# iris1997jiatong/I-DCCRN-VAE

Measured on AMD Instinct MI355X. Metric: 4s@16kHz utterances/sec fwd+SI-SNR, DCCRN-CL, 1/2/4/8 MI355X vs host CPU, higher is better.
Workload: dtype f32; 1 GPU; supervised DCCRN-CL forward(train=False) + final_ete_loss (weights 0/0/1); batch_per_gpu=64, utterance=4 s @ 16 kHz (64000 samples, 641 frames), parallelism=replicas x1, streams=1, input=resident in HBM

## Files before the change

### i-dccrn-vae_amd/csrc/cgemm_tw.hip

```cpp
#include <atomic>
#include <cstdint>
#include <cstdlib>
#include <type_traits>
#include "cgemm.hpp"
#include "conv_epilogue.hpp"
#include "cgemm_tw_map.hpp"
#include "../../include/idccrn_hip.h"

namespace {

struct TwArgs {
    const float* x0;
    const float* x1;
    int C0, C1;
    int Fin, Fout;
    int J, Jp, Tp;
    const float* wfrag;
    int UP;
    const float* epi;
    int has_fold;
    const float* slope;
    float* out;
    int Cout, cotiles;
    int tshift, t_valid;
    double* stats;
    int stats_rep;
    const float* add;
    int add_div, add_Jp;
    TwGrid grid;
    int stagger;
};

constexpr int TW_PACK_CI = 8;
constexpr int TW_XCD_SPLIT = 1;
constexpr int TW_PAIR_STAGGER = 1;

template <int PH> __device__ __forceinline__ int tw_ra(int r) {
    if (PH == 0) return r == 0 ? 0 : (r == 2 ? 2 : 1);
    return r == 0 ? 1 : 2;
}
template <int PH> __device__ __forceinline__ int tw_rb(int r) {
    if (PH == 0) return r == 2 ? 1 : (r == 3 ? 3 : 2);
    return r == 0 ? 2 : 3;
}
template <int PH> __device__ __forceinline__ float tw_cb(int r) {
    if (PH == 0) return r == 1 ? 1.f : -1.f;
    return r == 1 ? 0.f : -1.f;
}
template <int PH> constexpr int tw_nr() { return PH == 0 ? 4 : 3; }
template <int PH> constexpr int tw_nt() { return tw_nr<PH>() * 9; }
template <int PH> constexpr int tw_ntp() { return PH == 0 ? 36 : 32; }
template <int PH> constexpr int tw_ntw() { return (tw_nt<PH>() + 3) / 4; }
__host__ __device__ inline int tw_tile(int ph, int w, int k) {
    if (ph == 0) return w * 9 + k;
    if (w < 3) return k < 6 ? w * 9 + k : w * 9 + 8;
    return k < 6 ? (k >> 1) * 9 + 6 + (k & 1) : -1;
}
template <int PH> constexpr int tw_wslots() { return PH == 0 ? 9 : 8; }

template <int PH, int CIK, bool LEFT, bool STATS = false, int NCT = 1>
__global__ __launch_bounds__(256 * NCT, NCT == 1 ? 2 : 1) void cconv_tw_kernel(const TwArgs a) {
    constexpr int NR = tw_nr<PH>(), NT = tw_nt<PH>(), NTP = tw_ntp<PH>(), NTW = tw_ntw<PH>();
    constexpr int NRAW = PH == 0 ? 4 : 3, ROW0 = PH == 0 ? 0 : 1;
    constexpr int KS = CIK / 2;
    constexpr int RT = NRAW * 9 * 32;
    constexpr int NE = CIK * RT;
    constexpr int NBUF = 2;
    constexpr int RDW = 2;
    constexpr bool STAGE_BEHIND_W = PH == 0 && NCT == 2;
    constexpr int NITEM = CIK * NRAW * 16;
    constexpr int NTHR = 256 * NCT;
    constexpr int NLD = (NITEM + NTHR - 1) / NTHR;
    static_assert(NCT == 1 || NCT == 2, "one or two co tiles per workgroup");
    static_assert(KS % RDW == 0 && NLD <= 2, "weight ring slots are compile-time; at most two staging items per thread");
    static_assert(NLD + NCT - 1 < KS, "the staging k-steps (from 1 on, waves 4 .. 7 one later) end before the barrier's k-step");
    static_assert(NCT * NT * 4 * 64 <= NBUF * NE, "the epilogue exchange (one area per co tile) fits the patch buffers");

    extern __shared__ __attribute__((aligned(16))) float smem[];

    const int tid = threadIdx.x;
    const int lane = tid & 63;
    const int wave = __builtin_amdgcn_readfirstlane(tid >> 6);
    const int w4 = NCT == 1 ? wave : wave & 3, cth = NCT == 1 ? 0 : wave >> 2;
    const int half = lane >> 5, l31 = lane & 31;

    TwTile tile;
    if (!tw_block_tile(a.grid, blockIdx.x, tile)) return;
    const bool edge = PH == 0 && tile.edge;
    const int jt = tile.jt, ft = tile.ft;
    int ct = tile.ct;
    ct = NCT * ct + cth;
    const int j0 = jt * 64;
    const int m0 = 2 * ft;
    const int rbase = m0 - 1 + ROW0;

    const int Cin = a.C0 + a.C1;
    const int nchunk = (Cin + CIK - 1) / CIK;

    f32x16 acc[NTW];
#pragma unroll
    for (int k = 0; k < NTW; ++k)
#pragma unroll
        for (int r = 0; r < 16; ++r) acc[k][r] = 0.f;
    constexpr int NPAIR = (NTW - 1) / 2;
    constexpr bool UNI = PH == 0;
    int offA[UNI ? 1 : NPAIR + 1], offB[UNI ? 1 : NPAIR + 1];
    float cbj[UNI ? 1 : NPAIR + 1];
    if (UNI) {
        cbj[0] = edge ? 0.f : tw_cb<PH>(w4);
        offA[0] = (edge ? w4 : tw_ra<PH>(w4) - ROW0) * 288;
        offB[0] = (edge ? w4 : tw_rb<PH>(w4) - ROW0) * 288;
    } else {
#pragma unroll
        for (int j = 0; j <= NPAIR; ++j) {
            int t = tw_tile(PH, w4, j < NPAIR ? 2 * j : NTW - 1);
            t = t < 0 ? 0 : t;
            const int r = t / 9, plane = t - r * 9;
            cbj[j] = tw_cb<PH>(r);
            const int po = plane == 8 ? 256 : (plane >> 1) * 64;
            offA[j] = (tw_ra<PH>(r) - ROW0) * 288 + po;
            offB[j] = cbj[j] != 0.f ? (tw_rb<PH>(r) - ROW0) * 288 + po : offA[j];
        }
    }

    f32x4 v_r[NLD], v_i[NLD];
    float e_r[NLD], e_i[NLD];
    unsigned off_v[NLD], off_e[NLD], ldsoff[NLD];
    unsigned okmask[NLD];
    int item_cl[NLD];
    bool interior[NLD];
#pragma unroll
    for (int i = 0; i < NLD; ++i) {
        const int e = tid + i * NTHR;
        const int c8 = e & 15;
        const int rl = (e >> 4) % NRAW, cl = e / (16 * NRAW);
        item_cl[i] = cl;
        const int f = edge ? a.Fin - 2 + (rl & 1) : rbase + rl;
        const int jc = j0 + (edge ? 64 * (rl >> 1) : 0) + 4 * c8;
        const int je = LEFT ? jc - 1 : jc + 4;
        const bool exists = e < NITEM;
        const bool okr = exists && f >= 0 && f < a.Fin;
        unsigned m = 0;
#pragma unroll
        for (int q = 0; q < 5; ++q) {
            const int c = jc + q + (LEFT ? -1 : 0);
            if (c >= 0 && c < a.J) m |= 1u << q;
        }
        if (okr) m |= 1u << 5;
        if (exists) m |= 1u << 7;
        const int jcv = jc + 3 < a.Jp ? jc : 0;
        const int jev = (je >= 0 && je < a.Jp) ? je : 0;
        off_v[i] = okr ? (unsigned)((cl * a.Fin + f) * a.Jp + jcv) : 0u;
        off_e[i] = okr ? (unsigned)((cl * a.Fin + f) * a.Jp + jev) : 0u;
        if (jc + 3 >= a.Jp) m &= ~0x1fu;
        if (!(je >= 0 && je < a.Jp)) m &= LEFT ? ~1u : ~(1u << 4);
        okmask[i] = m;
        interior[i] = __builtin_amdgcn_ballot_w64((m & 0xbfu) == 0xbfu) == ~0ull;
        ldsoff[i] = (unsigned)((cl * NRAW + rl) * 288 + 4 * c8);
    }
    auto stage_load = [&](int chunk, int i) {
        const int ci0 = chunk * CIK;
        const bool from0 = ci0 < a.C0;
        const float* br = from0 ? a.x0 + (size_t)ci0 * a.Fin * a.Jp : a.x1 + (size_t)(ci0 - a.C0) * a.Fin * a.Jp;
        const float* bi = from0 ? br + (size_t)a.C0 * a.Fin * a.Jp : br + (size_t)a.C1 * a.Fin * a.Jp;
        const int cvalid = (from0 ? a.C0 : Cin) - ci0;
        const bool dead = item_cl[i] >= cvalid;
        const unsigned ov = dead ? 0u : off_v[i], oe = dead ? 0u : off_e[i];
        v_r[i] = *(const f32x4*)(br + ov);
        v_i[i] = *(const f32x4*)(bi + ov);
        e_r[i] = br[oe];
        e_i[i] = bi[oe];
    };
    float fr[5], fi[5];
    auto stage_window = [&](int chunk, int i) {
        const int ci0s = chunk * CIK;
        const int cvalid = (ci0s < a.C0 ? a.C0 : Cin) - ci0s;
        constexpr bool left = LEFT;
        if (interior[i] && cvalid >= CIK) {
#pragma unroll
            for (int q = 0; q < 5; ++q) {
                fr[q] = left ? (q == 0 ? e_r[i] : v_r[i][q == 0 ? 0 : q - 1]) : (q == 4 ? e_r[i] : v_r[i][q == 4 ? 3 : q]);
                fi[q] = left ? (q == 0 ? e_i[i] : v_i[i][q == 0 ? 0 : q - 1]) : (q == 4 ? e_i[i] : v_i[i][q == 4 ? 3 : q]);
            }
            return;
        }
        unsigned m = okmask[i];
        if (item_cl[i] >= cvalid || !((m >> 5) & 1u)) m &= ~0x1fu;
#pragma unroll
        for (int q = 0; q < 5; ++q) {
            const float xr = left ? (q == 0 ? e_r[i] : v_r[i][q == 0 ? 0 : q - 1]) : (q == 4 ? e_r[i] : v_r[i][q == 4 ? 3 : q]);
            const float xi = left ? (q == 0 ? e_i[i] : v_i[i][q == 0 ? 0 : q - 1]) : (q == 4 ? e_i[i] : v_i[i][q == 4 ? 3 : q]);
            const bool cok = (m >> q) & 1u;
            fr[q] = cok ? xr : 0.f;
            fi[q] = cok ? xi : 0.f;
        }
    };
    auto plane_val = [&](int gt, int pr) -> float {
        const int g = gt / 3, tau = gt - g * 3;
        const int q0 = 2 * pr;
        const float xa_ = g == 0 ? fr[q0] + fi[q0] : (g == 1 ? fr[q0] : fi[q0]);
        const float xb_ = g == 0 ? fr[q0 + 1] + fi[q0 + 1] : (g == 1 ? fr[q0 + 1] : fi[q0 + 1]);
        const float xd_ = g == 0 ? fr[q0 + 2] + fi[q0 + 2] : (g == 1 ? fr[q0 + 2] : fi[q0 + 2]);
        return tau == 0 ? xa_ - xb_ : (tau == 1 ? xb_ : xb_ - xd_);
    };
// ... 1 lines not shown
    auto stage_plane2 = [&](float* dst, int i, int j) {
        if (!item_exists(i)) return;
        if (j < 4) {
            f32x4 o = {plane_val(2 * j, 0), plane_val(2 * j + 1, 0), plane_val(2 * j, 1), plane_val(2 * j + 1, 1)};
            *(f32x4*)(dst + ldsoff[i] + j * 64) = o;
        } else {
            *(float2*)(dst + ldsoff[i] - 2 * (int)(tid & 15) + 256) = make_float2(plane_val(8, 0), plane_val(8, 1));
        }
    };
    auto stage_store = [&](float* dst, int chunk, int i) {
        stage_window(chunk, i);
#pragma unroll
        for (int j = 0; j < 5; ++j) stage_plane2(dst, i, j);
    };

    constexpr int WS = tw_wslots<PH>();
    constexpr int NWR = PH == 0 ? NTW : 8;
    const size_t wregion = PH == 1 ? (size_t)a.cotiles * a.UP * tw_ntp<0>() : (edge ? (size_t)a.cotiles * a.UP * (tw_ntp<0>() + tw_ntp<1>()) : 0);
    const float* wbase = a.wfrag + (wregion + (size_t)ct * a.UP * NTP) * 64 + (size_t)w4 * WS * 64;
    const int total_ks = nchunk * KS;
    float a_w[RDW][NWR];
    auto load_w = [&](int g, float (&dst)[NWR]) {
        g = g < total_ks ? g : total_ks - 1;
        const float* ws = wbase + (size_t)g * NTP * 64;
        const f32x4 w0 = *(const f32x4*)(ws + lane * 4), w1 = *(const f32x4*)(ws + 256 + lane * 4);
#pragma unroll
        for (int k = 0; k < 4; ++k) {
            dst[k] = w0[k];
            dst[4 + k] = w1[k];
        }
        if (NTW == 9) dst[NTW - 1] = ws[512 + lane];
    };
    float xa[NTW], xb[NTW];
    auto load_raw2 = [&](const float* base, int j) {
        if (j < NPAIR) {
            const int oa = UNI ? offA[0] + j * 64 : offA[UNI ? 0 : j], ob = UNI ? offB[0] + j * 64 : offB[UNI ? 0 : j];
            const float2 pa_ = *(const float2*)(base + oa + 2 * l31), pb_ = *(const float2*)(base + ob + 2 * l31);
            xa[2 * j] = pa_.x; xa[2 * j + 1] = pa_.y;
            xb[2 * j] = pb_.x; xb[2 * j + 1] = pb_.y;
        } else {
            xa[NTW - 1] = base[(UNI ? offA[0] + 256 : offA[UNI ? 0 : NPAIR]) + l31];
            xb[NTW - 1] = base[(UNI ? offB[0] + 256 : offB[UNI ? 0 : NPAIR]) + l31];
        }
    };
    auto load_raw_all = [&](const float* base) {
#pragma unroll
        for (int j = 0; j <= NPAIR; ++j) load_raw2(base, j);
    };

#pragma unroll
    for (int i = 0; i < NLD; ++i) stage_load(0, i);
#pragma unroll
    for (int u = 0; u < RDW; ++u) load_w(u, a_w[u]);
#pragma unroll
    for (int i = 0; i < NLD; ++i) stage_store(smem, 0, i);
#pragma unroll
    for (int i = 0; i < NLD; ++i) stage_load(nchunk > 1 ? 1 : 0, i);
    __syncthreads();

    load_raw_all(smem + (size_t)half * RT);
    auto run = [&](auto late_) {
        constexpr bool LATE = decltype(late_)::value;
        for (int chunk = 0; chunk < nchunk; ++chunk) {
            const float* P = smem + (chunk & 1) * NE;
            float* Pn = smem + ((chunk + 1) & 1) * NE;
            const int nxt = chunk + 1 < nchunk ? chunk + 1 : chunk, nxt2 = chunk + 2 < nchunk ? chunk + 2 : nchunk - 1;
#pragma unroll
            for (int ul = 0; ul < KS; ++ul) {
                const float* bnext = ul + 1 < KS ? P + (size_t)(2 * (ul + 1) + half) * RT : Pn + (size_t)half * RT;
                const int si = ul - 1 - (LATE ? 1 : 0);
                const bool staging = si >= 0 && si < NLD;
#pragma unroll
                for (int k = 0; k < NTW; ++k) {
                    const float b = xa[k] + cbj[UNI ? 0 : (k >> 1 < NPAIR ? k >> 1 : NPAIR)] * xb[k];
                    if (PH == 1 && k == 4)
                        asm volatile("" ::"v"(a_w[ul % RDW][4]), "v"(a_w[ul % RDW][5]), "v"(a_w[ul % RDW][6]), "v"(a_w[ul % RDW][7]));
                    acc[k] = __builtin_amdgcn_mfma_f32_32x32x2f32(a_w[ul % RDW][k], b, acc[k], 0, 0, 0);
                    if (ul == KS - 1 && k == 0) {
                        __builtin_amdgcn_sched_barrier(0);
                        __syncthreads();
                    }
                    if ((k & 1) && (k >> 1) < NPAIR) load_raw2(bnext, k >> 1);
                    if (k == NTW - 1) load_raw2(bnext, NPAIR);
                    if (staging) {
                        if (k == 0) stage_window(nxt, si);
                        if ((k & 1) && k < 6) stage_plane2(Pn, si, k >> 1);
                        if (k == (NTW == 9 ? 7 : 6)) stage_plane2(Pn, si, 3);
                        if (k == NTW - 1) stage_plane2(Pn, si, 4);
                        if (k == NTW - 1 && !STAGE_BEHIND_W) stage_load(nxt2, si);
                    }
                    __builtin_amdgcn_sched_barrier(0);
                }
                load_w(chunk * KS + ul + RDW, a_w[ul % RDW]);
                if (STAGE_BEHIND_W && staging) {
                    __builtin_amdgcn_sched_barrier(0);
                    stage_load(nxt2, si);
                }
            }
        }
    };
    if (NCT == 2 && PH == 1 && a.stagger && cth)
        run(std::integral_constant<bool, NCT == 2 && PH == 1>{});
    else
        run(std::false_type{});
    __syncthreads();

    const float slope = a.slope ? *a.slope : 1.0f;
    const bool has_act = a.slope != nullptr;
    float* E = smem + cth * (NT * 4 * 64);
    const int jAc[2] = {j0 + 2 * l31, j0 + 2 * l31 + (edge ? 64 : 0)};
    bool keep[2][2], inb[2][2];
    int ja[2][2];
#pragma unroll
    for (int c = 0; c < 2; ++c)
#pragma unroll
        for (int q = 0; q < 2; ++q) {
// ... 181 lines not shown
    const int cotiles = (Cout + 31) / 32;
    const int cpad = (cin_used + TW_PACK_CI - 1) / TW_PACK_CI * TW_PACK_CI;
    const long long n = idv_cconv_tw_wfrag_floats(Cout, cin_used);
    const unsigned blocks = (unsigned)((n + 255) / 256 > 4096 ? 4096 : (n + 255) / 256);
    hipLaunchKernelGGL(pack_cconv_tw_kernel, dim3(blocks), dim3(256), 0, (hipStream_t)stream, wino_frag, cotiles, cpad * 3, cpad / 2,
                       cin_used, tw_frag);
    return idv_launch_status();
}

extern "C" int idv_ctconv2d_tw_fwd(const float* x0, int C0, const float* x1, int C1, const float* wfrag, const float* epi, int has_fold,
                                   const float* prelu_slope, float* out, double* stats, double* stats_work, int stats_rep, int tshift,
                                   int Cout, int Fin, int B, int Tp, int Jp, int t_valid_out, const float* addend, int addend_div,
                                   int addend_Jp, void* stream) {
    if (!x0 || !wfrag || !epi || !out || C0 <= 0 || Cout <= 0 || Fin <= 0 || B <= 0 || Tp <= 1) return IDV_EINVAL;
    const EpiStatsTarget sums{stats, stats_work, stats_rep};
    if (!sums.ok()) return IDV_EINVAL;
    if (addend && (addend_div < 1 || B % addend_div || addend_Jp < (B / addend_div) * Tp)) return IDV_EINVAL;
    if (C1 > 0 && !x1) return IDV_EINVAL;
    if (tshift != 0 && tshift != -1) return IDV_EINVAL;
    if (!idv_cconv_tw_supported(C0, C1, Cout, Fin)) return IDV_EINVAL;
    if ((Jp & 3) || (reinterpret_cast<uintptr_t>(x0) & 15) || (C1 > 0 && (reinterpret_cast<uintptr_t>(x1) & 15)) ||
        (reinterpret_cast<uintptr_t>(out) & 7))
        return IDV_EINVAL;
    TwArgs a{};
    a.x0 = x0; a.x1 = x1; a.C0 = C0; a.C1 = C1;
    a.Fin = Fin; a.Fout = 2 * Fin - 1;
    a.J = B * Tp; a.Jp = Jp; a.Tp = Tp;
    a.wfrag = wfrag; a.UP = (C0 + C1 + TW_PACK_CI - 1) / TW_PACK_CI * TW_PACK_CI / 2;
    a.epi = epi; a.has_fold = has_fold; a.slope = prelu_slope; a.out = out;
    a.Cout = Cout; a.cotiles = (Cout + 31) / 32;
    a.tshift = tshift; a.t_valid = t_valid_out;
    a.add = addend; a.add_div = addend ? addend_div : 1; a.add_Jp = addend_Jp;
    if (Jp < a.J) return IDV_EINVAL;
    if ((long long)8 * Fin * (long long)Jp >= 0xffffffffLL) return IDV_EINVAL;
    hipStream_t st = (hipStream_t)stream;
    sums.set(a);
    int rc = 0;
    rc = launch_tw_ph<0, 8>(a, st);
    if (!rc) rc = launch_tw_ph<1, 8>(a, st);
    return sums.finish(rc, Cout, st);
}
```

### i-dccrn-vae_amd/csrc/cgemm_tw2.hip

```cpp
#include <cstdint>
#include <cstdlib>
#include <type_traits>
#include "cgemm.hpp"
#include "conv_epilogue.hpp"
#include "cgemm_tw_map.hpp"
#include "../../include/idccrn_hip.h"

namespace {

typedef f32x4 f32x4_a4 __attribute__((aligned(4)));

struct Tw2Args {
    const float* x0;
    int Cin;
    int Fin, Fout;
    int J, Jp, Tp;
    const float* wfrag;
    int UP;
    const float* epi;
    int has_fold;
    const float* slope;
    float* out;
    int Cout, cotiles;
    int tshift, t_valid;
    double* stats;
    int stats_rep;
    TwGrid grid;
    int stagger;
};

constexpr int TW2_PACK_CI = 8;
constexpr int TW2_XCD_SPLIT = 1;
constexpr int TW2_PAIR_STAGGER = 1;

__host__ __device__ constexpr int tw2_ra(int q) { return q == 0 ? 0 : (q == 1 ? 2 : (q == 2 ? 4 : (q == 3 ? 2 : (q == 4 ? 1 : 3)))); }
__host__ __device__ constexpr int tw2_rb(int q) { return q == 0 ? 4 : (q == 1 ? 4 : (q == 2 ? 2 : (q == 3 ? 6 : (q == 4 ? 3 : (q == 5 ? 3 : 5))))); }
__host__ __device__ constexpr float tw2_cb(int q) { return q == 1 ? 1.f : (q == 5 ? 0.f : -1.f); }
__host__ __device__ constexpr int tw2_qx(int a) { return a == 0 ? 0 : (a == 1 ? 1 : 3); }
__host__ __device__ constexpr int tw2_qy(int a) { return a == 0 ? 4 : (a == 1 ? 5 : 6); }
__host__ __device__ constexpr int tw2_main_acc(int w) { return w == 2 ? 3 : w; }
__host__ __device__ inline void tw2_slot(int w, int k, int& q, int& plane) {
// ... 51 lines not shown

    const int tid = threadIdx.x;
    const int lane = tid & 63;
    const int wave = __builtin_amdgcn_readfirstlane(tid >> 6);
    const int w4 = NCT == 1 ? wave : wave & 3, cth = NCT == 1 ? 0 : wave >> 2;
    const int half = lane >> 5, l31 = lane & 31;

    TwTile tile;
    if (!tw_block_tile(a.grid, blockIdx.x, tile)) return;
    const bool edge = tile.edge;
    const int jt = tile.jt, ft = tile.ft;
    const int ct = NCT * tile.ct + cth;
    const int j0 = jt * 64;
    const int m0 = 2 * ft;
    const int rbase = 2 * m0 - 2;

    const int Cin = a.Cin;
    const int nchunk = (Cin + CIK - 1) / CIK;

    f32x16 acc[NACC];
#pragma unroll
    for (int k = 0; k < NACC; ++k)
#pragma unroll
        for (int r = 0; r < 16; ++r) acc[k][r] = 0.f;

    f32x4 v_r[NLD], v_i[NLD];
    float e_r[NLD], e_i[NLD];
    unsigned off_v[NLD], ldsoff[NLD];
    unsigned okmask[NLD];
    bool interior[NLD];
    auto item_cl = [&](int i) -> int { return (tid + i * NTHR) / (16 * NRAW); };
#pragma unroll
    for (int i = 0; i < NLD; ++i) {
        const int e = tid + i * NTHR;
        const int c8 = e & 15;
        const int cl = e / (16 * NRAW), rl = (NCT == 2 && e >= NITEM) ? 0 : (e >> 4) % NRAW;
        const int f = edge ? (rl < 6 ? a.Fin - 3 + rl % 3 : -1) : rbase + rl;
        const int jc = j0 + (edge && rl >= 3 ? 64 : 0) + 4 * c8;
        const int je = LEFT ? jc - 1 : jc + 4;
        const bool exists = e < NITEM;
        const bool okr = exists && f >= 0 && f < a.Fin;
        unsigned m = 0;
#pragma unroll
        for (int q = 0; q < 5; ++q) {
            const int c = jc + q + (LEFT ? -1 : 0);
            if (c >= 0 && c < a.J) m |= 1u << q;
        }
        if (okr) m |= 1u << 5;
        const int jcv = jc + 3 < a.Jp ? jc : 0;
        off_v[i] = okr ? (unsigned)((cl * a.Fin + f) * a.Jp + jcv) : 4u;
        if (jc + 3 >= a.Jp) m &= ~0x1fu;
        if (!(je >= 0 && je < a.Jp)) m &= LEFT ? ~1u : ~(1u << 4);
        okmask[i] = m;
        interior[i] = __builtin_amdgcn_ballot_w64((m & 0x3fu) == 0x3fu) == ~0ull;
        ldsoff[i] = (unsigned)((cl * NRAW + rl) * 288 + 4 * c8);
    }
    auto item_exists = [&](int i) -> bool { return i == 0 || wave * 64 + 256 < NITEM; };
    auto stage_load = [&](int chunk, int i) {
        if (!item_exists(i)) return;
        const int ci0 = chunk * CIK;
        const float* br = a.x0 + (size_t)ci0 * a.Fin * a.Jp;
        const float* bi = br + (size_t)Cin * a.Fin * a.Jp;
        const bool dead = item_cl(i) >= Cin - ci0;
        const unsigned ov = dead ? 4u : off_v[i];
        const float* pr = br + ov - (LEFT ? 1 : 0);
        const float* pi = bi + ov - (LEFT ? 1 : 0);
        using Win = std::conditional_t<LEFT, f32x4_a4, f32x4>;
        v_r[i] = *(const Win*)pr;
        v_i[i] = *(const Win*)pi;
        e_r[i] = pr[4];
        e_i[i] = pi[4];
    };
    float fr[5], fi[5];
    auto stage_window = [&](int chunk, int i) {
        if (!item_exists(i)) return;
        const int cvalid = Cin - chunk * CIK;
        if (interior[i] && cvalid >= CIK) {
#pragma unroll
            for (int q = 0; q < 5; ++q) {
                fr[q] = q == 4 ? e_r[i] : v_r[i][q == 4 ? 3 : q];
                fi[q] = q == 4 ? e_i[i] : v_i[i][q == 4 ? 3 : q];
            }
            return;
        }
        unsigned m = okmask[i];
        if (item_cl(i) >= cvalid || !((m >> 5) & 1u)) m &= ~0x1fu;
#pragma unroll
        for (int q = 0; q < 5; ++q) {
            const float xr = q == 4 ? e_r[i] : v_r[i][q == 4 ? 3 : q];
            const float xi = q == 4 ? e_i[i] : v_i[i][q == 4 ? 3 : q];
            const bool cok = (m >> q) & 1u;
            fr[q] = cok ? xr : 0.f;
            fi[q] = cok ? xi : 0.f;
        }
    };
    auto plane_val = [&](int gt, int pr) -> float {
        const int g = gt / 3, tau = gt - g * 3;
        const int q0 = 2 * pr;
        const float xa_ = g == 0 ? fr[q0] + fi[q0] : (g == 1 ? fr[q0] : fi[q0]);
// ... 2 lines not shown
        return tau == 0 ? xa_ - xb_ : (tau == 1 ? xb_ : xb_ - xd_);
    };
    auto stage_plane2 = [&](float* dst, int i, int j) {
        if (!item_exists(i)) return;
        if (j < 4) {
            f32x4 o = {plane_val(2 * j, 0), plane_val(2 * j + 1, 0), plane_val(2 * j, 1), plane_val(2 * j + 1, 1)};
            *(f32x4*)(dst + ldsoff[i] + j * 64) = o;
        } else {
            *(float2*)(dst + ldsoff[i] - 2 * (int)(tid & 15) + 256) = make_float2(plane_val(8, 0), plane_val(8, 1));
        }
    };
    auto stage_store = [&](float* dst, int chunk, int i) {
        stage_window(chunk, i);
#pragma unroll
        for (int j = 0; j < 5; ++j) stage_plane2(dst, i, j);
    };

    const float* wbase = a.wfrag + (((size_t)(edge ? a.cotiles : 0) + ct) * a.UP * 4 + w4) * 1024 + lane * 4;
    const int total_ks = nchunk * KS;
    float a_w[NSLOT];
    auto load_wg = [&](int g, int grp) {
        g = g < total_ks ? g : total_ks - 1;
        const f32x4 w4 = *(const f32x4*)(wbase + (size_t)g * 4096 + grp * 256);
#pragma unroll
        for (int k = 0; k < 4; ++k) a_w[grp * 4 + k] = w4[k];
    };

    const int am = tw2_main_acc(w4 < 3 ? w4 : 0);
    const int qxm = tw2_qx(am), qym = tw2_qy(am);
    const int rxa = tw2_ra(qxm) * 288, rxb = tw2_rb(qxm) * 288, rya = tw2_ra(qym) * 288, ryb = tw2_rb(qym) * 288;
    const float cbx = tw2_cb(qxm), cby = tw2_cb(qym);
    const int r2a = tw2_ra(2) * 288 + w4 * 64, r2b = tw2_rb(2) * 288 + w4 * 64;
    float xa[2][4], xb[2][4];
    auto load_grp_a = [&](const float* base, int g, float (&oa)[4], float (&ob)[4]) {
        if (g < 3) {
            const float2 xa_ = *(const float2*)(base + rxa + g * 64 + 2 * l31), xb_ = *(const float2*)(base + rxb + g * 64 + 2 * l31);
            const float2 ya_ = *(const float2*)(base + rya + g * 64 + 2 * l31), yb_ = *(const float2*)(base + ryb + g * 64 + 2 * l31);
            oa[0] = xa_.x; oa[2] = xa_.y; ob[0] = xb_.x; ob[2] = xb_.y;
            oa[1] = ya_.x; oa[3] = ya_.y; ob[1] = yb_.x; ob[3] = yb_.y;
        } else {
            oa[0] = base[rxa + 3 * 64 + 2 * l31]; ob[0] = base[rxb + 3 * 64 + 2 * l31];
            oa[1] = base[rya + 3 * 64 + 2 * l31]; ob[1] = base[ryb + 3 * 64 + 2 * l31];
            const float2 pa_ = *(const float2*)(base + r2a + 2 * l31), pb_ = *(const float2*)(base + r2b + 2 * l31);
            oa[2] = pa_.x; oa[3] = pa_.y; ob[2] = pb_.x; ob[3] = pb_.y;
        }
    };
    auto load_grp_b = [&](const float* base, int g, float (&oa)[4], float (&ob)[4]) {
#pragma unroll
        for (int s4 = 0; s4 < 4; ++s4) {
            int q, plane;
            tw2_slot(3, 4 * g + s4, q, plane);
            if (q < 0) continue;
            oa[s4] = base[tw2_ra(q) * 288 + tw2_poff(plane, l31)];
            ob[s4] = base[tw2_rb(q) * 288 + tw2_poff(plane, l31)];
        }
    };
    const int eoff = (w4 >> 1) * 3 * 288;
    auto load_grp_e = [&](auto odd_, const float* base, int g, float (&oa)[4]) {
#pragma unroll
        for (int s4 = 0; s4 < 4; ++s4) {
            int t, plane;
            if (!tw2_eslot(decltype(odd_)::value, 4 * g + s4, t, plane)) continue;
            oa[s4] = base[eoff + t * 288 + tw2_poff(plane, l31)];
        }
    };

    auto prologue = [&]() {
#pragma unroll
        for (int i = 0; i < NLD; ++i) stage_load(0, i);
#pragma unroll
        for (int grp = 0; grp < 4; ++grp) load_wg(0, grp);
#pragma unroll
        for (int i = 0; i < NLD; ++i) stage_store(smem, 0, i);
#pragma unroll
        for (int i = 0; i < NLD; ++i) stage_load(nchunk > 1 ? 1 : 0, i);
        __syncthreads();
    };

    auto run = [&](auto role, auto late_) {
        constexpr int ROLE = decltype(role)::value;
        constexpr bool ROLE_B = ROLE == 1, EDGE = ROLE >= 2;
        using EdgeOdd = std::integral_constant<bool, ROLE == 3>;
        prologue();
        if constexpr (EDGE) load_grp_e(EdgeOdd{}, smem + (size_t)half * RT, 0, xa[0]);
        else if (ROLE_B) load_grp_b(smem + (size_t)half * RT, 0, xa[0], xb[0]);
        else load_grp_a(smem + (size_t)half * RT, 0, xa[0], xb[0]);
        for (int chunk = 0; chunk < nchunk; ++chunk) {
            const float* P = smem + (chunk & 1) * NEB;
            float* Pn = smem + ((chunk + 1) & 1) * NEB;
            const int nxt = chunk + 1 < nchunk ? chunk + 1 : chunk, nxt2 = chunk + 2 < nchunk ? chunk + 2 : nchunk - 1;
#pragma unroll
            for (int ul = 0; ul < KS; ++ul) {
                const float* bnext = ul + 1 < KS ? P + (size_t)(2 * (ul + 1) + half) * RT : Pn + (size_t)half * RT;
                const bool staging = ul == 0;
#pragma unroll
                for (int k = 0; k < (ROLE_B ? NSLOT - 1 : NSLOT); ++k) {
                    const int g = k >> 2, s4 = k & 3;
                    float cb;
                    int ai;
                    bool product = true;
                    if (EDGE) {
                        int t, plane;
                        product = tw2_eslot(EdgeOdd::value, k, t, plane);
                        cb = 0.f;
                        ai = plane - (EdgeOdd::value ? 5 : 0);
                    } else if (ROLE_B) {
                        int q, plane;
                        tw2_slot(3, k, q, plane);
                        cb = tw2_cb(q);
                        ai = k < 12 ? k >> 1 : 6 + (k - 12);
                    } else {
                        cb = k < 14 ? ((k & 1) ? cby : cbx) : -1.f;
                        ai = k < 14 ? k >> 1 : 7 + (k - 14);
                    }
                    if ((ROLE_B || EDGE) && s4 == 0) asm volatile("" ::"v"(a_w[k]), "v"(a_w[k + 1]), "v"(a_w[k + 2]), "v"(a_w[k + 3]));
                    if (s4 == 0) {
                        const float* src = g < 3 ? P + (size_t)(2 * ul + half) * RT : bnext;
                        if (!(ul == KS - 1 && g == 3)) {
                            if constexpr (EDGE) load_grp_e(EdgeOdd{}, src, (g + 1) & 3, xa[(g + 1) & 1]);
                            else if (ROLE_B) load_grp_b(src, (g + 1) & 3, xa[(g + 1) & 1], xb[(g + 1) & 1]);
                            else load_grp_a(src, (g + 1) & 3, xa[(g + 1) & 1], xb[(g + 1) & 1]);
                        }
                    }
                    if constexpr (EDGE) {
                        if (product) acc[ai] = __builtin_amdgcn_mfma_f32_32x32x2f32(a_w[k], xa[g & 1][s4], acc[ai], 0, 0, 0);
                    } else {
                        const float b = xa[g & 1][s4] + cb * xb[g & 1][s4];
                        acc[ai] = __builtin_amdgcn_mfma_f32_32x32x2f32(a_w[k], b, acc[ai], 0, 0, 0);
                    }
                    if (ul == KS - 1 && k == 0) {
                        __builtin_amdgcn_sched_barrier(0);
                        __syncthreads();
                    }
                    if (ul == KS - 1 && k == 12) {
                        if constexpr (EDGE) load_grp_e(EdgeOdd{}, bnext, 0, xa[0]);
                        else if (ROLE_B) load_grp_b(bnext, 0, xa[0], xb[0]);
                        else load_grp_a(bnext, 0, xa[0], xb[0]);
                    }
                    if ((k & 3) == 3 || (ROLE_B && k == NSLOT - 2)) load_wg(chunk * KS + ul + 1, k >> 2);
                    if constexpr (NCT == 2) if (staging) {
                        constexpr bool late = decltype(late_)::value;
                        if (k <= 5 && !late) {
                            if (k == 0) stage_window(nxt, 0);
                            if (k >= 1) stage_plane2(Pn, 0, k - 1);
                            if (k == 5) stage_load(nxt2, 0);
                        }
                        if (k >= 8 && k <= 13 && late) {
                            if (k == 8) stage_window(nxt, 0);
                            if (k >= 9) stage_plane2(Pn, 0, k - 9);
                            if (k == 13) stage_load(nxt2, 0);
                        }
                    }
                    if constexpr (NCT == 1) if (staging) {
                        if (k == 0) stage_window(nxt, 0);
                        if (k >= 1 && k <= 5) stage_plane2(Pn, 0, k - 1);
                        if (k == 5) stage_load(nxt2, 0);
                        if (!ROLE_B) {
                            if (k == 8) stage_window(nxt, 1);
                            if (k >= 9 && k <= 13) stage_plane2(Pn, 1, k - 9);
                            if (k == 13) stage_load(nxt2, 1);
                        }
                    }
                    __builtin_amdgcn_sched_barrier(0);
                }
            }
        }
    };
    using Late = std::integral_constant<bool, NCT == 2>;
    const bool late = NCT == 2 && a.stagger && cth;
    if (edge) {
// ... 163 lines not shown
    const long long cotiles = (Cout + 31) / 32, cpad = (cin_used + TW2_PACK_CI - 1) / TW2_PACK_CI * TW2_PACK_CI;
    return cotiles * (cpad / 2) * 2 * 4096;
}

extern "C" int idv_pack_cconv_tw2(const float* wino_frag, int Cout, int cin_used, float* tw_frag, void* stream) {
    if (!wino_frag || !tw_frag || Cout <= 0 || cin_used <= 0) return IDV_EINVAL;
    const int cotiles = (Cout + 31) / 32;
    const int cpad = (cin_used + TW2_PACK_CI - 1) / TW2_PACK_CI * TW2_PACK_CI;
    const long long n = idv_cconv_tw2_wfrag_floats(Cout, cin_used);
    const unsigned blocks = (unsigned)((n + 255) / 256 > 4096 ? 4096 : (n + 255) / 256);
    hipLaunchKernelGGL(pack_cconv_tw2_kernel, dim3(blocks), dim3(256), 0, (hipStream_t)stream, wino_frag, cotiles, cpad * 3, cpad / 2,
                       tw_frag);
    return idv_launch_status();
}

extern "C" int idv_cconv2d_tw_fwd(const float* x0, int Cin, const float* wfrag, const float* epi, int has_fold, const float* prelu_slope,
                                  float* out, double* stats, double* stats_work, int stats_rep, int tshift, int Cout, int Fin, int B, int Tp,
                                  int Jp, int t_valid_out, void* stream) {
    if (!x0 || !wfrag || !epi || !out || Cin <= 0 || Cout <= 0 || Fin <= 0 || B <= 0 || Tp <= 1) return IDV_EINVAL;
    const EpiStatsTarget sums{stats, stats_work, stats_rep};
    if (!sums.ok()) return IDV_EINVAL;
    if (tshift != 0 && tshift != -1) return IDV_EINVAL;
    if (!idv_cconv_tw2_supported(Cin, Cout, Fin)) return IDV_EINVAL;
    if ((Jp & 3) || (reinterpret_cast<uintptr_t>(x0) & 15) || (reinterpret_cast<uintptr_t>(out) & 7)) return IDV_EINVAL;
    Tw2Args a{};
    a.x0 = x0; a.Cin = Cin;
    a.Fin = Fin; a.Fout = (Fin - 1) / 2 + 1;
    a.J = B * Tp; a.Jp = Jp; a.Tp = Tp;
    a.wfrag = wfrag; a.UP = (Cin + TW2_PACK_CI - 1) / TW2_PACK_CI * TW2_PACK_CI / 2;
    a.epi = epi; a.has_fold = has_fold; a.slope = prelu_slope; a.out = out;
    a.Cout = Cout; a.cotiles = (Cout + 31) / 32;
    a.tshift = tshift; a.t_valid = t_valid_out;
    if (Jp < a.J) return IDV_EINVAL;
    if ((long long)4 * Fin * (long long)Jp >= 0xffffffffLL) return IDV_EINVAL;
    hipStream_t st = (hipStream_t)stream;
    sums.set(a);
    int rc;
    const bool pair = a.cotiles % 2 == 0 && (idv_tw_pair(-1) & IDV_TW_PAIR_CONV);
    switch ((stats ? 4 : 0) | (pair ? 2 : 0) | (tshift ? 1 : 0)) {
        case 0: rc = launch_tw2<false, false, 1>(a, st); break;
        case 1: rc = launch_tw2<true, false, 1>(a, st); break;
        case 2: rc = launch_tw2<false, false, 2>(a, st); break;
        case 3: rc = launch_tw2<true, false, 2>(a, st); break;
        case 4: rc = launch_tw2<false, true, 1>(a, st); break;
        case 5: rc = launch_tw2<true, true, 1>(a, st); break;
        case 6: rc = launch_tw2<false, true, 2>(a, st); break;
        default: rc = launch_tw2<true, true, 2>(a, st); break;
    }
    return sums.finish(rc, Cout, st);
}
```

Before: 1059 utterances/sec.

## Use precomputed LDS base pointers, byte offsets, and one-ahead B-operand transform in tw conv kernels

The complex conv kernels now keep per-lane LDS base pointers in address space 3 and flip them between the two buffers, so operand reads can use immediate offsets instead of recomputing addresses each k-step. Global staging offsets are precomputed in bytes through a shared helper, which drops a shift per load. The B operand (xa + cb*xb) is computed one MFMA ahead so the VALU work overlaps the matrix pipe. The cost is more live registers and tighter range checks on host-side offsets.

```diff
diff --git a/i-dccrn-vae_amd/csrc/cgemm_tw.hip b/i-dccrn-vae_amd/csrc/cgemm_tw.hip
--- a/i-dccrn-vae_amd/csrc/cgemm_tw.hip
+++ b/i-dccrn-vae_amd/csrc/cgemm_tw.hip
@@ -5,9 +5,14 @@
 #include "cgemm.hpp"
 #include "conv_epilogue.hpp"
 #include "cgemm_tw_map.hpp"
+#include "cgemm_tw_stage.hpp"
 #include "../../include/idccrn_hip.h"
 
 namespace {
+
+typedef __attribute__((address_space(3))) float LdsF;
+typedef float TwF2 __attribute__((ext_vector_type(2)));
+typedef __attribute__((address_space(3))) TwF2 LdsF2;
 
 struct TwArgs {
     const float* x0;
@@ -68,6 +73,7 @@
     constexpr int NBUF = 2;
     constexpr int RDW = 2;
     constexpr bool STAGE_BEHIND_W = PH == 0 && NCT == 2;
+    constexpr bool KBASE = !(PH == 1 && NCT == 1);
     constexpr int NITEM = CIK * NRAW * 16;
     constexpr int NTHR = 256 * NCT;
     constexpr int NLD = (NITEM + NTHR - 1) / NTHR;
@@ -131,32 +137,13 @@
     bool interior[NLD];
 #pragma unroll
     for (int i = 0; i < NLD; ++i) {
-        const int e = tid + i * NTHR;
-        const int c8 = e & 15;
-        const int rl = (e >> 4) % NRAW, cl = e / (16 * NRAW);
-        item_cl[i] = cl;
-        const int f = edge ? a.Fin - 2 + (rl & 1) : rbase + rl;
-        const int jc = j0 + (edge ? 64 * (rl >> 1) : 0) + 4 * c8;
-        const int je = LEFT ? jc - 1 : jc + 4;
-        const bool exists = e < NITEM;
-        const bool okr = exists && f >= 0 && f < a.Fin;
-        unsigned m = 0;
-#pragma unroll
-        for (int q = 0; q < 5; ++q) {
-            const int c = jc + q + (LEFT ? -1 : 0);
-            if (c >= 0 && c < a.J) m |= 1u << q;
-        }
-        if (okr) m |= 1u << 5;
-        if (exists) m |= 1u << 7;
-        const int jcv = jc + 3 < a.Jp ? jc : 0;
-        const int jev = (je >= 0 && je < a.Jp) ? je : 0;
-        off_v[i] = okr ? (unsigned)((cl * a.Fin + f) * a.Jp + jcv) : 0u;
-        off_e[i] = okr ? (unsigned)((cl * a.Fin + f) * a.Jp + jev) : 0u;
-        if (jc + 3 >= a.Jp) m &= ~0x1fu;
-        if (!(je >= 0 && je < a.Jp)) m &= LEFT ? ~1u : ~(1u << 4);
-        okmask[i] = m;
-        interior[i] = __builtin_amdgcn_ballot_w64((m & 0xbfu) == 0xbfu) == ~0ull;
-        ldsoff[i] = (unsigned)((cl * NRAW + rl) * 288 + 4 * c8);
+        const TwStageItem it = tw_stage_item(tid + i * NTHR, NRAW, NITEM, LEFT, edge, a.Fin, a.J, a.Jp, j0, rbase, KBASE ? 4u : 1u);
+        item_cl[i] = it.cl;
+        off_v[i] = it.off_v;
+        off_e[i] = it.off_e;
+        okmask[i] = it.mask;
+        interior[i] = __builtin_amdgcn_ballot_w64((it.mask & 0xbfu) == 0xbfu) == ~0ull;
+        ldsoff[i] = it.ldsoff;
     }
     auto stage_load = [&](int chunk, int i) {
         const int ci0 = chunk * CIK;
@@ -165,11 +152,18 @@
         const float* bi = from0 ? br + (size_t)a.C0 * a.Fin * a.Jp : br + (size_t)a.C1 * a.Fin * a.Jp;
         const int cvalid = (from0 ? a.C0 : Cin) - ci0;
         const bool dead = item_cl[i] >= cvalid;
-        const unsigned ov = dead ? 0u : off_v[i], oe = dead ? 0u : off_e[i];
-        v_r[i] = *(const f32x4*)(br + ov);
-        v_i[i] = *(const f32x4*)(bi + ov);
-        e_r[i] = br[oe];
-        e_i[i] = bi[oe];
+        const unsigned ov = dead ? 4u * TW_DUMMY : off_v[i], oe = dead ? 4u * TW_DUMMY : off_e[i];
+        if constexpr (KBASE) {
+            v_r[i] = *(const f32x4*)((const char*)br + ov);
+            v_i[i] = *(const f32x4*)((const char*)bi + ov);
+            e_r[i] = *(const float*)((const char*)br + oe);
+            e_i[i] = *(const float*)((const char*)bi + oe);
+        } else {
+            v_r[i] = *(const f32x4*)(br + ov);
+            v_i[i] = *(const f32x4*)(bi + ov);
+            e_r[i] = br[oe];
+            e_i[i] = bi[oe];
+        }
     };
     float fr[5], fi[5];
     auto stage_window = [&](int chunk, int i) {
@@ -237,7 +231,43 @@
         if (NTW == 9) dst[NTW - 1] = ws[512 + lane];
     };
     float xa[NTW], xb[NTW];
-    auto load_raw2 = [&](const float* base, int j) {
+    constexpr int NBASE = UNI ? 2 : NPAIR + 1;
+    const LdsF* pA[NBASE];
+    const LdsF* pB[NBASE];
+    {
+        const LdsF* s0 = (const LdsF*)smem + half * RT;
+#pragma unroll
+        for (int j = 0; j < NBASE; ++j) {
+            const bool single = j == NBASE - 1;
+            const int lp = single ? (UNI ? 256 : 0) + l31 : 2 * l31;
+            pA[j] = s0 + offA[UNI ? 0 : j] + lp;
+            pB[j] = s0 + offB[UNI ? 0 : j] + lp;
+        }
+    }
+    static_assert(NE + (2 * (KS - 1) + 1) * RT + (NRAW - 1) * 288 + 256 + 31 < NBUF * NE, "operand reads stay inside the LDS allocation");
+    static_assert(((2 * (KS - 1)) * RT + (NPAIR - 1) * 64) * 4 < 65536, "k-step and plane-pair offsets fit the LDS read's immediate");
+    static_assert(NBUF == 2, "the bases alternate between two buffers");
+    int flip = NE;
+    auto flip_bases = [&]() {
+#pragma unroll
+        for (int j = 0; j < NBASE; ++j) {
+            pA[j] += flip;
+            pB[j] += flip;
+        }
+        flip = -flip;
+    };
+    auto load_raw2 = [&](int koff, int j) {
+        if (j < NPAIR) {
+            const int po = koff + (UNI ? j * 64 : 0);
+            const TwF2 pa_ = *(const LdsF2*)(pA[UNI ? 0 : j] + po), pb_ = *(const LdsF2*)(pB[UNI ? 0 : j] + po);
+            xa[2 * j] = pa_.x; xa[2 * j + 1] = pa_.y;
+            xb[2 * j] = pb_.x; xb[2 * j + 1] = pb_.y;
+        } else {
+            xa[NTW - 1] = pA[NBASE - 1][koff];
+            xb[NTW - 1] = pB[NBASE - 1][koff];
+        }
+    };
+    auto load_raw2_p = [&](const float* base, int j) {
         if (j < NPAIR) {
             const int oa = UNI ? offA[0] + j * 64 : offA[UNI ? 0 : j], ob = UNI ? offB[0] + j * 64 : offB[UNI ? 0 : j];
             const float2 pa_ = *(const float2*)(base + oa + 2 * l31), pb_ = *(const float2*)(base + ob + 2 * l31);
@@ -248,10 +278,14 @@
             xb[NTW - 1] = base[(UNI ? offB[0] + 256 : offB[UNI ? 0 : NPAIR]) + l31];
         }
     };
-    auto load_raw_all = [&](const float* base) {
-#pragma unroll
-        for (int j = 0; j <= NPAIR; ++j) load_raw2(base, j);
-    };
+    auto load_raw_all = [&]() {
+#pragma unroll
+        for (int j = 0; j <= NPAIR; ++j) {
+            if constexpr (KBASE) load_raw2(0, j);
+            else load_raw2_p(smem + (size_t)half * RT, j);
+        }
+    };
+    auto xform = [&](int k) -> float { return xa[k] + cbj[UNI ? 0 : (k >> 1 < NPAIR ? k >> 1 : NPAIR)] * xb[k]; };
 
 #pragma unroll
     for (int i = 0; i < NLD; ++i) stage_load(0, i);
@@ -263,7 +297,8 @@
     for (int i = 0; i < NLD; ++i) stage_load(nchunk > 1 ? 1 : 0, i);
     __syncthreads();
 
-    load_raw_all(smem + (size_t)half * RT);
+    load_raw_all();
+    float bcur = KBASE ? xform(0) : 0.f;
     auto run = [&](auto late_) {
         constexpr bool LATE = decltype(late_)::value;
         for (int chunk = 0; chunk < nchunk; ++chunk) {
@@ -272,21 +307,35 @@
             const int nxt = chunk + 1 < nchunk ? chunk + 1 : chunk, nxt2 = chunk + 2 < nchunk ? chunk + 2 : nchunk - 1;
 #pragma unroll
             for (int ul = 0; ul < KS; ++ul) {
-                const float* bnext = ul + 1 < KS ? P + (size_t)(2 * (ul + 1) + half) * RT : Pn + (size_t)half * RT;
+                const int bnext = ul + 1 < KS ? 2 * (ul + 1) * RT : 0;
+                const float* bnext_p = ul + 1 < KS ? P + (size_t)(2 * (ul + 1) + half) * RT : Pn + (size_t)half * RT;
+                auto load_next = [&](int j) {
+                    if constexpr (KBASE) load_raw2(bnext, j);
+                    else load_raw2_p(bnext_p, j);
+                };
                 const int si = ul - 1 - (LATE ? 1 : 0);
                 const bool staging = si >= 0 && si < NLD;
 #pragma unroll
                 for (int k = 0; k < NTW; ++k) {
-                    const float b = xa[k] + cbj[UNI ? 0 : (k >> 1 < NPAIR ? k >> 1 : NPAIR)] * xb[k];
+                    float bn = 0.f;
+                    if constexpr (KBASE) {
+                        bn = xform(k + 1 < NTW ? k + 1 : 0);
+                        if (PH == 1) asm volatile("" : "+v"(bn));
+                        __builtin_amdgcn_sched_barrier(0);
+                    } else {
+                        bcur = xform(k);
+                    }
                     if (PH == 1 && k == 4)
                         asm volatile("" ::"v"(a_w[ul % RDW][4]), "v"(a_w[ul % RDW][5]), "v"(a_w[ul % RDW][6]), "v"(a_w[ul % RDW][7]));
-                    acc[k] = __builtin_amdgcn_mfma_f32_32x32x2f32(a_w[ul % RDW][k], b, acc[k], 0, 0, 0);
+                    acc[k] = __builtin_amdgcn_mfma_f32_32x32x2f32(a_w[ul % RDW][k], bcur, acc[k], 0, 0, 0);
+                    if constexpr (KBASE) bcur = bn;
                     if (ul == KS - 1 && k == 0) {
                         __builtin_amdgcn_sched_barrier(0);
                         __syncthreads();
+                        if constexpr (KBASE) flip_bases();
                     }
-                    if ((k & 1) && (k >> 1) < NPAIR) load_raw2(bnext, k >> 1);
-                    if (k == NTW - 1) load_raw2(bnext, NPAIR);
+                    if ((k & 1) && (k >> 1) < NPAIR) load_next(k >> 1);
+                    if (k == NTW - 1) load_next(NPAIR);
                     if (staging) {
                         if (k == 0) stage_window(nxt, si);
                         if ((k & 1) && k < 6) stage_plane2(Pn, si, k >> 1);
@@ -534,7 +583,7 @@
     a.tshift = tshift; a.t_valid = t_valid_out;
     a.add = addend; a.add_div = addend ? addend_div : 1; a.add_Jp = addend_Jp;
     if (Jp < a.J) return IDV_EINVAL;
-    if ((long long)8 * Fin * (long long)Jp >= 0xffffffffLL) return IDV_EINVAL;
+    if ((long long)4 * 8 * Fin * (long long)Jp >= 0xffffffffLL) return IDV_EINVAL;
     hipStream_t st = (hipStream_t)stream;
     sums.set(a);
     int rc = 0;
diff --git a/i-dccrn-vae_amd/csrc/cgemm_tw2.hip b/i-dccrn-vae_amd/csrc/cgemm_tw2.hip
--- a/i-dccrn-vae_amd/csrc/cgemm_tw2.hip
+++ b/i-dccrn-vae_amd/csrc/cgemm_tw2.hip
@@ -4,9 +4,14 @@
 #include "cgemm.hpp"
 #include "conv_epilogue.hpp"
 #include "cgemm_tw_map.hpp"
+#include "cgemm_tw_stage.hpp"
 #include "../../include/idccrn_hip.h"
 
 namespace {
+
+typedef __attribute__((address_space(3))) float LdsF;
+typedef float TwF2 __attribute__((ext_vector_type(2)));
+typedef __attribute__((address_space(3))) TwF2 LdsF2;
 
 typedef f32x4 f32x4_a4 __attribute__((aligned(4)));
 
@@ -124,28 +129,11 @@
     auto item_cl = [&](int i) -> int { return (tid + i * NTHR) / (16 * NRAW); };
 #pragma unroll
     for (int i = 0; i < NLD; ++i) {
-        const int e = tid + i * NTHR;
-        const int c8 = e & 15;
-        const int cl = e / (16 * NRAW), rl = (NCT == 2 && e >= NITEM) ? 0 : (e >> 4) % NRAW;
-        const int f = edge ? (rl < 6 ? a.Fin - 3 + rl % 3 : -1) : rbase + rl;
-        const int jc = j0 + (edge && rl >= 3 ? 64 : 0) + 4 * c8;
-        const int je = LEFT ? jc - 1 : jc + 4;
-        const bool exists = e < NITEM;
-        const bool okr = exists && f >= 0 && f < a.Fin;
-        unsigned m = 0;
-#pragma unroll
-        for (int q = 0; q < 5; ++q) {
-            const int c = jc + q + (LEFT ? -1 : 0);
-            if (c >= 0 && c < a.J) m |= 1u << q;
-        }
-        if (okr) m |= 1u << 5;
-        const int jcv = jc + 3 < a.Jp ? jc : 0;
-        off_v[i] = okr ? (unsigned)((cl * a.Fin + f) * a.Jp + jcv) : 4u;
-        if (jc + 3 >= a.Jp) m &= ~0x1fu;
-        if (!(je >= 0 && je < a.Jp)) m &= LEFT ? ~1u : ~(1u << 4);
-        okmask[i] = m;
-        interior[i] = __builtin_amdgcn_ballot_w64((m & 0x3fu) == 0x3fu) == ~0ull;
-        ldsoff[i] = (unsigned)((cl * NRAW + rl) * 288 + 4 * c8);
+        const TwStageItem it = tw2_stage_item(tid + i * NTHR, NITEM, NCT == 2, LEFT, edge, a.Fin, a.J, a.Jp, j0, rbase);
+        off_v[i] = it.off_v;
+        okmask[i] = it.mask;
+        interior[i] = __builtin_amdgcn_ballot_w64((it.mask & 0x3fu) == 0x3fu) == ~0ull;
+        ldsoff[i] = it.ldsoff;
     }
     auto item_exists = [&](int i) -> bool { return i == 0 || wave * 64 + 256 < NITEM; };
     auto stage_load = [&](int chunk, int i) {
@@ -154,9 +142,9 @@
         const float* br = a.x0 + (size_t)ci0 * a.Fin * a.Jp;
         const float* bi = br + (size_t)Cin * a.Fin * a.Jp;
         const bool dead = item_cl(i) >= Cin - ci0;
-        const unsigned ov = dead ? 4u : off_v[i];
-        const float* pr = br + ov - (LEFT ? 1 : 0);
-        const float* pi = bi + ov - (LEFT ? 1 : 0);
+        const unsigned ov = dead ? 4u * TW2_DUMMY : off_v[i];
+        const float* pr = (const float*)((const char*)br + ov) - (LEFT ? 1 : 0);
+        const float* pi = (const float*)((const char*)bi + ov) - (LEFT ? 1 : 0);
         using Win = std::conditional_t<LEFT, f32x4_a4, f32x4>;
         v_r[i] = *(const Win*)pr;
         v_i[i] = *(const Win*)pi;
@@ -225,16 +213,21 @@
     const float cbx = tw2_cb(qxm), cby = tw2_cb(qym);
     const int r2a = tw2_ra(2) * 288 + w4 * 64, r2b = tw2_rb(2) * 288 + w4 * 64;
     float xa[2][4], xb[2][4];
-    auto load_grp_a = [&](const float* base, int g, float (&oa)[4], float (&ob)[4]) {
+    static_assert(tw2_ra(tw2_qy(tw2_main_acc(0))) == tw2_ra(tw2_qx(tw2_main_acc(0))) + 1 &&
+                  tw2_ra(tw2_qy(tw2_main_acc(1))) == tw2_ra(tw2_qx(tw2_main_acc(1))) + 1 &&
+                  tw2_ra(tw2_qy(tw2_main_acc(2))) == tw2_ra(tw2_qx(tw2_main_acc(2))) + 1, "row ya = row xa + 1");
+    static_assert(KS == 2, "one xa / ya base per k-step");
+    auto load_grp_a = [&](const LdsF* const* pb, int koff, int g, float (&oa)[4], float (&ob)[4]) {
+        const LdsF* px = koff ? pb[2] + (koff - 2 * RT) : pb[0];
         if (g < 3) {
-            const float2 xa_ = *(const float2*)(base + rxa + g * 64 + 2 * l31), xb_ = *(const float2*)(base + rxb + g * 64 + 2 * l31);
-            const float2 ya_ = *(const float2*)(base + rya + g * 64 + 2 * l31), yb_ = *(const float2*)(base + ryb + g * 64 + 2 * l31);
+            const TwF2 xa_ = *(const LdsF2*)(px + g * 64), xb_ = *(const LdsF2*)(pb[1] + koff + g * 64);
+            const TwF2 ya_ = *(const LdsF2*)(px + 288 + g * 64), yb_ = *(const LdsF2*)(pb[3] + koff + g * 64);
             oa[0] = xa_.x; oa[2] = xa_.y; ob[0] = xb_.x; ob[2] = xb_.y;
             oa[1] = ya_.x; oa[3] = ya_.y; ob[1] = yb_.x; ob[3] = yb_.y;
         } else {
-            oa[0] = base[rxa + 3 * 64 + 2 * l31]; ob[0] = base[rxb + 3 * 64 + 2 * l31];
-            oa[1] = base[rya + 3 * 64 + 2 * l31]; ob[1] = base[ryb + 3 * 64 + 2 * l31];
-            const float2 pa_ = *(const float2*)(base + r2a + 2 * l31), pb_ = *(const float2*)(base + r2b + 2 * l31);
+            oa[0] = px[3 * 64]; ob[0] = pb[1][koff + 3 * 64];
+            oa[1] = px[288 + 3 * 64]; ob[1] = pb[3][koff + 3 * 64];
+            const TwF2 pa_ = *(const LdsF2*)(pb[4] + koff), pb_ = *(const LdsF2*)(pb[4] + koff + (tw2_rb(2) - tw2_ra(2)) * 288);
             oa[2] = pa_.x; oa[3] = pa_.y; ob[2] = pb_.x; ob[3] = pb_.y;
         }
     };
@@ -249,14 +242,30 @@
         }
     };
     const int eoff = (w4 >> 1) * 3 * 288;
-    auto load_grp_e = [&](auto odd_, const float* base, int g, float (&oa)[4]) {
+    auto load_grp_e = [&](auto odd_, const LdsF* const* pb, int koff, int g, float (&oa)[4]) {
 #pragma unroll
         for (int s4 = 0; s4 < 4; ++s4) {
-            int t, plane;
+            int t, plane, t2 = -1, plane2 = -1;
             if (!tw2_eslot(decltype(odd_)::value, 4 * g + s4, t, plane)) continue;
-            oa[s4] = base[eoff + t * 288 + tw2_poff(plane, l31)];
-        }
-    };
+            const bool two = s4 < 3 && tw2_eslot(decltype(odd_)::value, 4 * g + s4 + 1, t2, plane2) && t2 == t && !(plane & 1) &&
+                             plane2 == plane + 1 && plane2 < 8;
+            const bool second = s4 > 0 && tw2_eslot(decltype(odd_)::value, 4 * g + s4 - 1, t2, plane2) && t2 == t && (plane & 1) &&
+                                plane2 == plane - 1 && plane < 8;
+            if (second) continue;
+            if (two) {
+                const TwF2 v = *(const LdsF2*)(pb[0] + koff + t * 288 + (plane >> 1) * 64);
+                oa[s4] = v.x;
+                oa[s4 + 1] = v.y;
+            } else {
+                oa[s4] = pb[plane < 8 ? 0 : 1][koff + t * 288 + (plane < 8 ? (plane >> 1) * 64 + (plane & 1) : 256)];
+            }
+        }
+    };
+    static_assert(NEB + (2 * (KS - 1) + 1) * RT + 6 * 288 + 3 * 64 + 2 * 31 + 1 < 2 * NEB, "operand reads stay inside the LDS allocation");
+    static_assert((2 * (KS - 1) * RT + 6 * 288 + 256) * 4 < 65536, "k-step, row and plane offsets fit the LDS read's immediate");
+    static_assert(NEB + (2 * (KS - 1) + 1) * RT + (3 + 2) * 288 + 256 + 31 < 2 * NEB, "edge-wave reads stay inside the LDS allocation");
+    static_assert(NEB + (2 * (KS - 1) + 1) * RT + 6 * 288 + 256 + 31 < 2 * NEB, "wave 3's reads stay inside the LDS allocation");
+    static_assert(tw2_rb(6) <= 6 && tw2_rb(3) <= 6 && tw2_ra(2) <= 6, "raw rows 0 .. 6");
 
     auto prologue = [&]() {
 #pragma unroll
@@ -275,60 +284,92 @@
         constexpr bool ROLE_B = ROLE == 1, EDGE = ROLE >= 2;
         using EdgeOdd = std::integral_constant<bool, ROLE == 3>;
         prologue();
-        if constexpr (EDGE) load_grp_e(EdgeOdd{}, smem + (size_t)half * RT, 0, xa[0]);
-        else if (ROLE_B) load_grp_b(smem + (size_t)half * RT, 0, xa[0], xb[0]);
-        else load_grp_a(smem + (size_t)half * RT, 0, xa[0], xb[0]);
+        constexpr bool AHEAD = !EDGE && !ROLE_B;
+        constexpr bool BASES = !ROLE_B;
+        constexpr int NB = EDGE ? 2 : (BASES ? 5 : 1);
+        const LdsF* pb[NB];
+        if constexpr (EDGE) {
+            pb[0] = (const LdsF*)smem + half * RT + eoff + 2 * l31;
+            pb[1] = (const LdsF*)smem + half * RT + eoff + l31;
+        } else if constexpr (BASES) {
+            const int ro[5] = {rxa, rxb, rxa + 2 * RT, ryb, r2a};
+#pragma unroll
+            for (int j = 0; j < 5; ++j) pb[j] = (const LdsF*)smem + half * RT + ro[j] + 2 * l31;
+        }
+        int flip = NEB;
+        const float* Pcur = smem;
+        auto load_grp = [&](int koff, int g) {
+            if constexpr (EDGE) load_grp_e(EdgeOdd{}, pb, koff, g, xa[g & 1]);
+            else if constexpr (ROLE_B) load_grp_b(Pcur + (size_t)(koff / RT + half) * RT, g, xa[g & 1], xb[g & 1]);
+            else load_grp_a(pb, koff, g, xa[g & 1], xb[g & 1]);
+        };
+        auto xform = [&](int k) -> float {
+            float cb;
+            if constexpr (ROLE_B) {
+                int q, plane;
+                tw2_slot(3, k, q, plane);
+                cb = tw2_cb(q);
+            } else {
+                cb = k < 14 ? ((k & 1) ? cby : cbx) : -1.f;
+            }
+            return xa[(k >> 2) & 1][k & 3] + cb * xb[(k >> 2) & 1][k & 3];
+        };
+        constexpr int NK = ROLE_B ? NSLOT - 1 : NSLOT;
+        load_grp(0, 0);
+        float bcur = 0.f;
+        if constexpr (AHEAD) bcur = xform(0);
         for (int chunk = 0; chunk < nchunk; ++chunk) {
-            const float* P = smem + (chunk & 1) * NEB;
             float* Pn = smem + ((chunk + 1) & 1) * NEB;
+            if constexpr (ROLE_B) Pcur = smem + (chunk & 1) * NEB;
             const int nxt = chunk + 1 < nchunk ? chunk + 1 : chunk, nxt2 = chunk + 2 < nchunk ? chunk + 2 : nchunk - 1;
 #pragma unroll
             for (int ul = 0; ul < KS; ++ul) {
-                const float* bnext = ul + 1 < KS ? P + (size_t)(2 * (ul + 1) + half) * RT : Pn + (size_t)half * RT;
                 const bool staging = ul == 0;
 #pragma unroll
-                for (int k = 0; k < (ROLE_B ? NSLOT - 1 : NSLOT); ++k) {
+                for (int k = 0; k < NK; ++k) {
                     const int g = k >> 2, s4 = k & 3;
-                    float cb;
                     int ai;
                     bool product = true;
                     if (EDGE) {
                         int t, plane;
                         product = tw2_eslot(EdgeOdd::value, k, t, plane);
-                        cb = 0.f;
                         ai = plane - (EdgeOdd::value ? 5 : 0);
                     } else if (ROLE_B) {
-                        int q, plane;
-                        tw2_slot(3, k, q, plane);
-                        cb = tw2_cb(q);
                         ai = k < 12 ? k >> 1 : 6 + (k - 12);
                     } else {
-                        cb = k < 14 ? ((k & 1) ? cby : cbx) : -1.f;
                         ai = k < 14 ? k >> 1 : 7 + (k - 14);
+                    }
+                    float bn = 0.f;
+                    if constexpr (AHEAD) {
+                        bn = xform(k + 1 < NK ? k + 1 : 0);
+                        asm volatile("" : "+v"(bn));
+                        __builtin_amdgcn_sched_barrier(0);
                     }
                     if ((ROLE_B || EDGE) && s4 == 0) asm volatile("" ::"v"(a_w[k]), "v"(a_w[k + 1]), "v"(a_w[k + 2]), "v"(a_w[k + 3]));
                     if (s4 == 0) {
-                        const float* src = g < 3 ? P + (size_t)(2 * ul + half) * RT : bnext;
-                        if (!(ul == KS - 1 && g == 3)) {
-                            if constexpr (EDGE) load_grp_e(EdgeOdd{}, src, (g + 1) & 3, xa[(g + 1) & 1]);
-                            else if (ROLE_B) load_grp_b(src, (g + 1) & 3, xa[(g + 1) & 1], xb[(g + 1) & 1]);
-                            else load_grp_a(src, (g + 1) & 3, xa[(g + 1) & 1], xb[(g + 1) & 1]);
-                        }
+                        if (!(ul == KS - 1 && g == 3)) load_grp(g < 3 ? 2 * ul * RT : 2 * (ul + 1) * RT, (g + 1) & 3);
                     }
                     if constexpr (EDGE) {
                         if (product) acc[ai] = __builtin_amdgcn_mfma_f32_32x32x2f32(a_w[k], xa[g & 1][s4], acc[ai], 0, 0, 0);
+                    } else if constexpr (AHEAD) {
+                        acc[ai] = __builtin_amdgcn_mfma_f32_32x32x2f32(a_w[k], bcur, acc[ai], 0, 0, 0);
+                        bcur = bn;
                     } else {
-                        const float b = xa[g & 1][s4] + cb * xb[g & 1][s4];
-                        acc[ai] = __builtin_amdgcn_mfma_f32_32x32x2f32(a_w[k], b, acc[ai], 0, 0, 0);
+                        acc[ai] = __builtin_amdgcn_mfma_f32_32x32x2f32(a_w[k], xform(k), acc[ai], 0, 0, 0);
                     }
                     if (ul == KS - 1 && k == 0) {
                         __builtin_amdgcn_sched_barrier(0);
                         __syncthreads();
                     }
                     if (ul == KS - 1 && k == 12) {
-                        if constexpr (EDGE) load_grp_e(EdgeOdd{}, bnext, 0, xa[0]);
-                        else if (ROLE_B) load_grp_b(bnext, 0, xa[0], xb[0]);
-                        else load_grp_a(bnext, 0, xa[0], xb[0]);
+                        if constexpr (BASES) {
+#pragma unroll
+                            for (int j = 0; j < NB; ++j) pb[j] += flip;
+                            flip = -flip;
+                        } else {
+                            Pcur = Pn;
+                        }
+                        load_grp(0, 0);
                     }
                     if ((k & 3) == 3 || (ROLE_B && k == NSLOT - 2)) load_wg(chunk * KS + ul + 1, k >> 2);
                     if constexpr (NCT == 2) if (staging) {
@@ -558,7 +599,7 @@
     a.Cout = Cout; a.cotiles = (Cout + 31) / 32;
     a.tshift = tshift; a.t_valid = t_valid_out;
     if (Jp < a.J) return IDV_EINVAL;
-    if ((long long)4 * Fin * (long long)Jp >= 0xffffffffLL) return IDV_EINVAL;
+    if ((long long)4 * 4 * Fin * (long long)Jp >= 0xffffffffLL) return IDV_EINVAL;
     hipStream_t st = (hipStream_t)stream;
     sums.set(a);
     int rc;
diff --git a/i-dccrn-vae_amd/csrc/cgemm_tw_stage.hpp b/i-dccrn-vae_amd/csrc/cgemm_tw_stage.hpp
--- /dev/null
+++ b/i-dccrn-vae_amd/csrc/cgemm_tw_stage.hpp
@@ -0,0 +1,73 @@
+#pragma once
+
+#if defined(__HIPCC__) || defined(__CUDACC__)
+#define TW_SHD __host__ __device__
+#else
+#define TW_SHD
+#endif
+
+struct TwStageItem {
+    unsigned off_v, off_e;
+    unsigned ldsoff;
+    unsigned mask;
+    int cl;
+};
+
+constexpr unsigned TW_DUMMY = 0;
+constexpr unsigned TW2_DUMMY = 4;
+
+TW_SHD inline TwStageItem tw_stage_item(int e, int nraw, int nitem, bool left, bool edge, int Fin, int J, int Jp, int j0, int rbase,
+                                        unsigned unit) {
+    TwStageItem it;
+    const int c8 = e & 15;
+    const int rl = (e >> 4) % nraw, cl = e / (16 * nraw);
+    it.cl = cl;
+    const int f = edge ? Fin - 2 + (rl & 1) : rbase + rl;
+    const int jc = j0 + (edge ? 64 * (rl >> 1) : 0) + 4 * c8;
+    const int je = left ? jc - 1 : jc + 4;
+    const bool exists = e < nitem;
+    const bool okr = exists && f >= 0 && f < Fin;
+    unsigned m = 0;
+    for (int q = 0; q < 5; ++q) {
+        const int c = jc + q + (left ? -1 : 0);
+        if (c >= 0 && c < J) m |= 1u << q;
+    }
+    if (okr) m |= 1u << 5;
+    if (exists) m |= 1u << 7;
+    const int jcv = jc + 3 < Jp ? jc : 0;
+    const int jev = (je >= 0 && je < Jp) ? je : 0;
+    it.off_v = okr ? unit * (unsigned)((cl * Fin + f) * Jp + jcv) : unit * TW_DUMMY;
+    it.off_e = okr ? unit * (unsigned)((cl * Fin + f) * Jp + jev) : unit * TW_DUMMY;
+    if (jc + 3 >= Jp) m &= ~0x1fu;
+    if (!(je >= 0 && je < Jp)) m &= left ? ~1u : ~(1u << 4);
+    it.mask = m;
+    it.ldsoff = (unsigned)((cl * nraw + rl) * 288 + 4 * c8);
+    return it;
+}
+
+TW_SHD inline TwStageItem tw2_stage_item(int e, int nitem, bool dump, bool left, bool edge, int Fin, int J, int Jp, int j0, int rbase) {
+    constexpr int nraw = 7;
+    TwStageItem it;
+    const int c8 = e & 15;
+    const int cl = e / (16 * nraw), rl = (dump && e >= nitem) ? 0 : (e >> 4) % nraw;
+    it.cl = cl;
+    const int f = edge ? (rl < 6 ? Fin - 3 + rl % 3 : -1) : rbase + rl;
+    const int jc = j0 + (edge && rl >= 3 ? 64 : 0) + 4 * c8;
+    const int je = left ? jc - 1 : jc + 4;
+    const bool exists = e < nitem;
+    const bool okr = exists && f >= 0 && f < Fin;
+    unsigned m = 0;
+    for (int q = 0; q < 5; ++q) {
+        const int c = jc + q + (left ? -1 : 0);
+        if (c >= 0 && c < J) m |= 1u << q;
+    }
+    if (okr) m |= 1u << 5;
+    const int jcv = jc + 3 < Jp ? jc : 0;
+    it.off_v = okr ? 4u * (unsigned)((cl * Fin + f) * Jp + jcv) : 4u * TW2_DUMMY;
+    it.off_e = 0;
+    if (jc + 3 >= Jp) m &= ~0x1fu;
+    if (!(je >= 0 && je < Jp)) m &= left ? ~1u : ~(1u << 4);
+    it.mask = m;
+    it.ldsoff = (unsigned)((cl * nraw + rl) * 288 + 4 * c8);
+    return it;
+}
```

Result: faster. 1085 utterances/sec, median of 6 (+2.5%).
